# fergusfinn/qmps

Hardware: AMD Instinct MI355X
Metric: two-site energy evals/sec at D=4, batch=65536 (higher is better)
Workload: dtype f64

## Files before the change

### qmps_amd/csrc/qmps_direct.hip

```cpp
#include <hip/hip_runtime.h>
#include <stdint.h>

#include "qmps_hip.h"
#include "qmps_kernels.h"
#include "qmps_device.h"
#include "qmps_circuit.h"
#include "qmps_direct_core.h"
#include "qmps_direct_d8.h"

namespace qmps {

namespace {

struct QuadOps {
  using V = double;
  using P = bool;
  int q;
  const double2* row;
  double* gj;
  __device__ __forceinline__ P q_eq(int i) const { return q == i; }
  __device__ __forceinline__ P q_gt(int i) const { return q > i; }
  template <int L>
  static __device__ __forceinline__ V bcast(V v) { return quad_bcast<L>(v); }
  template <int L, int K>
  __device__ __forceinline__ void row_bcast(const V (&r)[16], V (&out)[16]) const {
#ifdef QMPS_GJ_LDS
    constexpr int K0 = K & ~1;
    __builtin_amdgcn_wave_barrier();
    if (q == L) {
#pragma unroll
      for (int j = K0; j < 16; j += 2) *(double2*)&gj[j] = make_double2(r[j], r[j + 1]);
    }
    __builtin_amdgcn_wave_barrier();
#pragma unroll
    for (int j = K0; j < 16; j += 2) {
      const double2 t = *(const double2*)&gj[j];
      if (j >= K) out[j] = t.x;
      out[j + 1] = t.y;
    }
#else
#pragma unroll
    for (int j = K; j < 16; ++j) out[j] = quad_bcast<L>(r[j]);
#endif
  }
  static __device__ __forceinline__ V qsum(V v) { return quad_sum(v); }
  static __device__ __forceinline__ V qmax(V v) {
    v = fmax(v, quad_perm<0xB1>(v));
    return fmax(v, quad_perm<0x4E>(v));
  }
  static __device__ __forceinline__ V vabs(V v) { return fabs(v); }
  static __device__ __forceinline__ V vmax(V a, V b) { return fmax(a, b); }
  static __device__ __forceinline__ V sel(P p, V a, V b) { return p ? a : b; }
  static __device__ __forceinline__ V splat(double x) { return x; }
  static __device__ __forceinline__ V fma(V a, V b, V c) { return dfma(a, b, c); }
  static __device__ __forceinline__ V rcp(V t) { return fast_rcp(t); }
  static __device__ __forceinline__ P lt(V a, V b) { return a < b; }
  static __device__ __forceinline__ P gt0(V a) { return a > 0.0; }
  static __device__ __forceinline__ P p_and(P a, P b) { return a && b; }
  static __device__ __forceinline__ P p_not(P a) { return !a; }
  static __device__ __forceinline__ bool any(P a) { return __any(a) != 0; }
  __device__ __forceinline__ void own(int s, int j, V& re, V& im) const {
    const double2 v = row[(4 * s + q) * 4 + j];
    re = v.x;
    im = v.y;
  }
  __device__ __forceinline__ void uni(int s, int i, int j, V& re, V& im) const {
    const double2 v = row[(4 * s + i) * 4 + j];
    re = v.x;
    im = v.y;
  }
  __device__ __forceinline__ void col(int s, int i, V& re, V& im) const {
    const double2 v = row[(4 * s + i) * 4 + q];
    re = v.x;
    im = v.y;
  }
};

typedef const __attribute__((address_space(4))) double* const_f64_ptr;
__device__ __forceinline__ const_f64_ptr h_term(const void* h, int t) { return (const_f64_ptr)(uintptr_t)h + 32 * t; }

typedef double v4f64 __attribute__((ext_vector_type(4)));
constexpr int kSqLD = 17;
constexpr int kSqDoubles = 16 * kSqLD + 16;

__device__ __forceinline__ void squaring_fallback(const unsigned char* tiles, int pad, double* img, int lane, bool todo,
                                                  int max_iter, double tol2, double (&x)[4], double& steps, bool& left) {
  constexpr int D = 4, LD = kSqLD;
  constexpr double RS2 = 0.70710678118654752, S2 = 1.4142135623730951;
  const int g = lane >> 4, c = lane & 15, j = c >> 2, jp = c & 3, q = lane & 3;
  double* strip = img + 16 * LD;
  const double cpx = j == jp ? 1.0 : (j < jp ? RS2 : 0.0), cpy = j > jp ? -RS2 : 0.0;
  const double cqx = j < jp ? RS2 : 0.0, cqy = j > jp ? RS2 : 0.0;
  const bool diag = j == jp;
  unsigned long long mask = __ballot(todo);
  while (mask != 0) {
    const int e = (__ffsll((long long)mask) - 1) >> 2;
    mask &= ~(0xFull << (4 * e));
    const double2* sA = (const double2*)(tiles + e * pad);
    v4f64 R;
    {
      double pr[2], pi[2], qr[2], qi[2];
#pragma unroll
      for (int s = 0; s < 2; ++s) {
        const double2 a = sA[(s * D + g) * D + jp], b = sA[(s * D + g) * D + j];
        pr[s] = dfma(cpx, a.x, cpy * a.y);
        pi[s] = dfma(cpy, a.x, -cpx * a.y);
        qr[s] = dfma(cqx, b.x, cqy * b.y);
        qi[s] = dfma(cqy, b.x, -cqx * b.y);
      }
#pragma unroll
      for (int reg = 0; reg < 4; ++reg) {
        double gr = 0.0, gi = 0.0;
#pragma unroll
        for (int s = 0; s < 2; ++s) {
          const double2 u = sA[(s * D + reg) * D + j], v = sA[(s * D + reg) * D + jp];
          gr = dfma(u.x, pr[s], gr);
          gr = dfma(-u.y, pi[s], gr);
          gr = dfma(v.x, qr[s], gr);
          gr = dfma(-v.y, qi[s], gr);
          gi = dfma(u.x, pi[s], gi);
          gi = dfma(u.y, pr[s], gi);
          gi = dfma(v.x, qi[s], gi);
          gi = dfma(v.y, qr[s], gi);
        }
        R[reg] = reg == g ? gr : (reg < g ? S2 * gr : -S2 * gi);
      }
    }
    double af[4];
    auto image = [&](const v4f64& M) {
      __builtin_amdgcn_wave_barrier();
#pragma unroll
      for (int reg = 0; reg < 4; ++reg) img[(4 * reg + g) * LD + c] = M[reg];
      __builtin_amdgcn_wave_barrier();
#pragma unroll
      for (int kk = 0; kk < 4; ++kk) af[kk] = img[c * LD + 4 * kk + g];
    };
    image(R);
    double prev = diag ? 0.25 : 0.0, z = prev, st = 0.0;
    bool active = true;
    int m = 0;
    while (active && m < 29 && (2 << m) <= max_iter) {
      v4f64 acc = {0.0, 0.0, 0.0, 0.0};
#pragma unroll
      for (int kk = 0; kk < 4; ++kk) acc = __builtin_amdgcn_mfma_f64_16x16x4f64(af[kk], R[kk], acc, 0, 0, 0);
      ++m;
      image(acc);
      z = 0.25 * ((img[c * LD + 0] + img[c * LD + 5]) + (img[c * LD + 10] + img[c * LD + 15]));
      const double inv = fast_rcp(row16_sum(diag ? z : 0.0));
      z *= inv;
      R = acc * inv;
#pragma unroll
      for (int kk = 0; kk < 4; ++kk) af[kk] *= inv;
      const double d = z - prev;
      const double d2 = row16_sum(d * d);
      prev = z;
      st = (double)(1 << m);
      active = !(d2 < tol2);
    }
    __builtin_amdgcn_wave_barrier();
    if (lane < 16) strip[lane] = diag ? z : RS2 * z;
    __builtin_amdgcn_wave_barrier();
    if ((lane >> 2) == e) {
      if (m > 0) {
#pragma unroll
        for (int l = 0; l < 4; ++l) x[l] = strip[4 * q + l];
      }
      steps = 1.0 + st;
      left = active;
    }
  }
}

}

#ifndef QMPS_DIRECT_MINWAVES
#define QMPS_DIRECT_MINWAVES 2
#endif
template <int ANS, bool WARM>
__global__ __launch_bounds__(64, QMPS_DIRECT_MINWAVES) void energy_direct_d4_kernel(LaneArgs p) {
  using Core = DirectD4<QuadOps>;
  constexpr int ROW = 512, PAD = ROW + 16, ITEMS = 16;
  __shared__ __attribute__((aligned(16))) unsigned char lds[ITEMS * PAD];
  __shared__ double sq_img[kSqDoubles];
#ifdef QMPS_GJ_LDS
  __shared__ __attribute__((aligned(16))) double gjbuf[ITEMS * 18];
#endif
  const int lane = threadIdx.x, e = lane >> 2, q = lane & 3;
  const int64_t first = (int64_t)blockIdx.x * ITEMS;
  const int64_t b = first + e;
  const bool valid = b < p.B;
  if constexpr (ANS >= 0) {
    Reg<3> reg;
#pragma unroll
    for (int xx = 0; xx < 8; ++xx) {
      reg.re[xx] = (valid && xx == q) ? 1.0 : 0.0;
      reg.im[xx] = 0.0;
    }
    const int nsh = p.ans_nsh;
    const int64_t row = valid ? b : 0;
    const int64_t ridx = nsh > 0 ? row / nsh : row;
    const int shift_k = nsh > 0 ? (int)(row - ridx * nsh) : 0;
    const int isel = nsh > 0 ? *p.ans_i : -1;
    const double* pp = p.ans_params + ridx * p.ans_P;
    constexpr int per = ANS == QMPS_ANSATZ_SHALLOW_CNOT3 ? 3 : 2, trip = ANS == QMPS_ANSATZ_SHALLOW_CNOT3 ? 3 : 4;
    const int P = p.ans_P;
    for (int l = 0; l + per <= P; l += trip) {
      const int mine = l + q;
      double ang = 0.0;
      if (q < trip && mine < P) {
        ang = pp[mine];
        if (mine == isel) ang += roto_shift_value(nsh, shift_k);
      }
      const double scale = ansatz_angle_scale<ANS>(ANS == QMPS_ANSATZ_SHALLOW_CNOT3 ? q : (q & 1));
      double sn, cs;
      sincos(scale * ang, &sn, &cs);
      {
        const double c0[3] = {quad_bcast<0>(cs), quad_bcast<1>(cs), quad_bcast<2>(cs)};
        const double s0[3] = {quad_bcast<0>(sn), quad_bcast<1>(sn), quad_bcast<2>(sn)};
        ansatz_layer_cs<3, ANS>(reg, c0, s0);
      }
      if (trip == 4 && l + 2 + per <= P) {
        const double c1[2] = {quad_bcast<2>(cs), quad_bcast<3>(cs)};
        const double s1[2] = {quad_bcast<2>(sn), quad_bcast<3>(sn)};
        ansatz_layer_cs<3, ANS>(reg, c1, s1);
      }
    }
    double2* tile = (double2*)(lds + e * PAD);
#pragma unroll
    for (int xx = 0; xx < 8; ++xx) tile[((xx & 1) * 4 + (xx >> 1)) * 4 + q] = make_double2(reg.re[xx], reg.im[xx]);
  } else {
    const unsigned char* slab = (const unsigned char*)p.A + first * ROW;
    const int64_t slab_bytes = (p.B - first < ITEMS ? p.B - first : ITEMS) * (int64_t)ROW;
    double2 v[ITEMS * ROW / 1024];
#pragma unroll
    for (int c = 0; c < ITEMS * ROW / 1024; ++c) {
      const int off = c * 1024 + lane * 16;
      v[c] = make_double2(0.0, 0.0);
      if (off < slab_bytes) v[c] = *(const double2*)(slab + off);
    }
#pragma unroll
    for (int c = 0; c < ITEMS * ROW / 1024; ++c) {
      const int off = c * 1024 + lane * 16;
      *(double2*)(lds + (off / ROW) * PAD + (off % ROW)) = v[c];
    }
  }
  __syncthreads();
#ifdef QMPS_GJ_LDS
  const QuadOps o{q, (const double2*)(lds + e * PAD), gjbuf + e * 18};
#else
  const QuadOps o{q, (const double2*)(lds + e * PAD), nullptr};
#endif
  const double tol2 = p.tol * p.tol;

  double x[4], us[16];
  double steps = 1.0;
  int status = QMPS_ST_OK;
  [[maybe_unused]] Core::SiteW W;
  bool have = false;
  if constexpr (WARM) {
    const double2* rin = (const double2*)p.r_in + (valid ? b : 0) * 16;
#pragma unroll
    for (int l = 0; l < 4; ++l) {
      const double2 rw = rin[q * 4 + l], cl = rin[l * 4 + q];
      x[l] = q <= l ? rw.x : cl.y;
    }
    Core::normalise(o, x);
    Core::gather(x, us);
    double y[4];
    const double d2 = Core::power_step(o, x, us, y);
    have = valid && d2 < tol2;
#pragma unroll
    for (int l = 0; l < 4; ++l) x[l] = have ? y[l] : x[l];
    __builtin_amdgcn_sched_barrier(0);
  }
  if (!WARM || __any(valid && !have)) {
    double Rc[4][16], xs[4], y[4];
    Core::build(o, Rc);
    __builtin_amdgcn_sched_barrier(0);
    double pivmax;
    Core::solve(o, Rc, xs, pivmax);
    __builtin_amdgcn_sched_barrier(0);
    Core::normalise(o, xs);
    Core::gather(xs, us);
    double d2;
    if constexpr (WARM) d2 = Core::power_step(o, xs, us, y);
    else d2 = Core::power_step_sites(o, xs, us, p.rho_need, y, W);
    __builtin_amdgcn_sched_barrier(0);
    const bool accepted = d2 < tol2 && pivmax < Core::kMaxInversePivot;
    if (!have) {
#pragma unroll
      for (int l = 0; l < 4; ++l) x[l] = xs[l];
      if (WARM) steps = 2.0;
    }
    const bool todo = valid && !have && !accepted;
    if (__any(todo)) {
      bool left = false;
      squaring_fallback(lds, PAD, sq_img, lane, todo, p.max_iter - 1, tol2, x, steps, left);
      if (__any(todo && left)) {
        double yb[4];
        Core::gather(x, us);
        const double d2b = Core::power_step(o, x, us, yb);
        const bool fin = todo && left && d2b < tol2 && steps + 1.0 <= (double)p.max_iter;
#pragma unroll
        for (int l = 0; l < 4; ++l) x[l] = fin ? yb[l] : x[l];
        if (fin) {
          left = false;
          steps += 1.0;
        }
      }
      if (todo) {
        status = left ? QMPS_ST_NOT_CONVERGED : QMPS_ST_OK;
        if (WARM) steps += 1.0;
      }
      if constexpr (!WARM) {
        Core::gather(x, us);
        Core::update_sites(o, us, p.rho_need, todo, W);
      }
    }
    if constexpr (WARM) Core::gather(x, us);
  } else {
    Core::gather(x, us);
  }
  __builtin_amdgcn_sched_barrier(0);

  double pre[4][4], pim[4][4];
  bool pd;
  if constexpr (WARM) pd = Core::density(o, us, p.rho_need, pre, pim);
  else pd = Core::density_sites(o, us, p.rho_need, W, pre, pim);
  if (status == QMPS_ST_OK && !pd) status = QMPS_ST_NOT_PD;
  if (p.acc_zero != nullptr && blockIdx.x == 0) acc_clear(p.acc_zero, p.n_terms, lane, 64);
  for (int t = 0; t < p.n_terms; ++t) {
    const double en = quad_sum(Core::energy(h_term(p.h, t), p.rho_need, pre, pim));
    if (valid && q == 0) p.E[b * p.n_terms + t] = en;
    if (p.partial != nullptr || p.acc != nullptr) {
      const double s = wave_sum((valid && q == 0) ? en : 0.0);
      if (lane == 0) {
        if (p.partial != nullptr) p.partial[(int64_t)t * gridDim.x + blockIdx.x] = s;
        if (p.acc != nullptr) acc_arrive(p.acc, p.acc_shards, t, blockIdx.x, s, p.acc_bound, p.acc_scale);
      }
    }
  }
  if (p.rho_out != nullptr) {
    double fre[4][4], fim[4][4];
#pragma unroll
    for (int t = 0; t < 4; ++t)
#pragma unroll
      for (int s = t; s < 4; ++s) {
        fre[t][s] = quad_sum(pre[t][s]);
        fim[t][s] = t == s ? 0.0 : quad_sum(pim[t][s]);
      }
    if (valid && q == 0) {
      double2* o2 = (double2*)p.rho_out + b * 16;
#pragma unroll
      for (int t = 0; t < 4; ++t)
#pragma unroll
        for (int s = 0; s < 4; ++s)
          o2[t * 4 + s] = t <= s ? make_double2(fre[t][s], fim[t][s]) : make_double2(fre[s][t], -fim[s][t]);
    }
  }
  if (!valid) return;
  if (q == 0) {
    p.iters[b] = (int32_t)steps;
    p.status[b] = status;
  }
  if (p.r_out != nullptr) {
    double2* o2 = (double2*)p.r_out + b * 16 + q * 4;
#pragma unroll
    for (int l = 0; l < 4; ++l) {
      const double f = q == 0 ? us[4 * l] : (q == 1 ? us[4 * l + 1] : (q == 2 ? us[4 * l + 2] : us[4 * l + 3]));
      const double re = q <= l ? x[l] : f;
      const double im = q == l ? 0.0 : (q < l ? f : -x[l]);
      o2[l] = make_double2(re, im);
    }
  }
}

#ifndef QMPS_ENERGY_ONLY_LEAN_WAVES
#define QMPS_ENERGY_ONLY_LEAN_WAVES 2
#endif
template <bool LEAN>
__global__ __launch_bounds__(64, LEAN ? QMPS_ENERGY_ONLY_LEAN_WAVES : 2) void energy_only_d4_kernel(LaneArgs p) {
  using Core = DirectD4<QuadOps>;
  constexpr int ROW = 512, PAD = ROW + 16, ITEMS = 16;
  __shared__ __attribute__((aligned(16))) unsigned char lds[ITEMS * PAD];
  const int lane = threadIdx.x, e = lane >> 2, q = lane & 3;
  const int64_t first = (int64_t)blockIdx.x * ITEMS;
  const int64_t b = first + e;
  const bool valid = b < p.B;
  if (p.acc_zero != nullptr && blockIdx.x == 0) acc_clear(p.acc_zero, p.n_terms, lane, 64);
  {
    const unsigned char* slab = (const unsigned char*)p.A + first * ROW;
    const int64_t slab_bytes = (p.B - first < ITEMS ? p.B - first : ITEMS) * (int64_t)ROW;
    double2 v[ITEMS * ROW / 1024];
#pragma unroll
    for (int c = 0; c < ITEMS * ROW / 1024; ++c) {
      const int off = c * 1024 + lane * 16;
      v[c] = make_double2(0.0, 0.0);
      if (off < slab_bytes) v[c] = *(const double2*)(slab + off);
    }
    double x[4];
    {
      const double2* rin = (const double2*)p.r_in + (valid ? b : 0) * 16;
#pragma unroll
      for (int l = 0; l < 4; ++l) {
        const double2 rw = rin[q * 4 + l], cl = rin[l * 4 + q];
        x[l] = q <= l ? rw.x : cl.y;
      }
    }
#pragma unroll
    for (int c = 0; c < ITEMS * ROW / 1024; ++c) {
      const int off = c * 1024 + lane * 16;
      *(double2*)(lds + (off / ROW) * PAD + (off % ROW)) = v[c];
    }
    __syncthreads();
    const QuadOps o{q, (const double2*)(lds + e * PAD), nullptr};
    Core::normalise(o, x);
    double us[16];
    double pre[4][4], pim[4][4], bre[4][4], bim[4][4];
    bool pd = true;
    if constexpr (LEAN) {
      Core::b_rows(o, bre, bim);
      Core::gather(x, us);
    } else {
      Core::gather(x, us);
      pd = Core::density(o, us, p.rho_need, pre, pim);
    }
    int status = QMPS_ST_OK;
    if (p.check_pd) {
      status = valid ? p.status[b] : QMPS_ST_OK;
      if (status == QMPS_ST_OK && !pd) status = QMPS_ST_NOT_PD;
    }
    for (int t = 0; t < p.n_terms; ++t) {
      double en;
      if constexpr (LEAN) en = quad_sum(Core::energy_lean(bre, bim, us, (const double*)p.h + 32 * t));
      else en = quad_sum(Core::energy(h_term(p.h, t), p.rho_need, pre, pim));
      if (valid && q == 0) p.E[b * p.n_terms + t] = en;
      if (p.partial != nullptr || p.acc != nullptr) {
        const double s = wave_sum((valid && q == 0) ? en : 0.0);
        if (lane == 0) {
          if (p.partial != nullptr) p.partial[(int64_t)t * gridDim.x + blockIdx.x] = s;
          if (p.acc != nullptr) acc_arrive(p.acc, p.acc_shards, t, blockIdx.x, s, p.acc_bound, p.acc_scale);
        }
      }
    }
    if (!LEAN && p.rho_out != nullptr) {
      double fre[4][4], fim[4][4];
#pragma unroll
      for (int t = 0; t < 4; ++t)
#pragma unroll
        for (int s2 = t; s2 < 4; ++s2) {
          fre[t][s2] = quad_sum(pre[t][s2]);
          fim[t][s2] = t == s2 ? 0.0 : quad_sum(pim[t][s2]);
        }
      if (valid && q == 0) {
        double2* o2 = (double2*)p.rho_out + b * 16;
#pragma unroll
        for (int t = 0; t < 4; ++t)
#pragma unroll
          for (int s2 = 0; s2 < 4; ++s2)
            o2[t * 4 + s2] = t <= s2 ? make_double2(fre[t][s2], fim[t][s2]) : make_double2(fre[s2][t], -fim[s2][t]);
      }
    }
    if (p.check_pd && valid && q == 0) p.status[b] = status;
  }
}

#ifndef QMPS_POWER_D4_MINWAVES
#define QMPS_POWER_D4_MINWAVES 4
#endif
template <int B, bool FRESH = false>
__device__ __forceinline__ void row_fmac(double& acc, double u, double m) {
  if constexpr (FRESH) asm("s_nop 1\n\tv_fmac_f64_dpp %0, %1, %2 row_newbcast:%3 row_mask:0xf bank_mask:0xf" : "+v"(acc) : "v"(u), "v"(m), "n"(B));
  else asm("v_fmac_f64_dpp %0, %1, %2 row_newbcast:%3 row_mask:0xf bank_mask:0xf" : "+v"(acc) : "v"(u), "v"(m), "n"(B));
}
template <bool GUESS>
__global__ __launch_bounds__(64, QMPS_POWER_D4_MINWAVES) void env_power_d4_kernel(LaneArgs p, int* __restrict__ counter, int first_block) {
  constexpr int PAD = 512 + 16, SLOTS = 4, kChunk = 8;
  __shared__ __attribute__((aligned(16))) unsigned char lds[SLOTS * PAD];
  const int lane = threadIdx.x, g = lane >> 4, c = lane & 15, i = c >> 2, ip = c & 3;
  const bool diag = i == ip, rot = i > ip;
  const double wt = diag ? 1.0 : 2.0;
  const double tol2 = p.tol * p.tol;
  const unsigned long long below = (1ull << (lane & ~15)) - 1ull;
  const double2* tile = (const double2*)(lds + g * PAD);
  int64_t b = 0;
  const int64_t dyn0 = (int64_t)gridDim.x * first_block;
  int64_t next = (int64_t)blockIdx.x * first_block, end = next + first_block;
  if (next > p.B) next = p.B;
  if (end > p.B) end = p.B;
  bool active = false, exhausted = dyn0 >= p.B;
  bool refill = true;
  int iters = 0;
  double u = 0.0, up = 0.0, R[16];
#pragma unroll
  for (int k = 0; k < 16; ++k) R[k] = 0.0;
  for (;;) {
    if (refill) {
      const unsigned long long idle = __ballot(!active);
      if (idle != 0ull && !(exhausted && next >= end)) {
        if (next >= end && !exhausted) {
          int base = 0;
          if (lane == 0) base = atomicAdd(counter, kChunk);
          const int64_t first = dyn0 + (int64_t)__builtin_amdgcn_readfirstlane(base);
          next = first < p.B ? first : p.B;
          end = first + kChunk < p.B ? first + kChunk : p.B;
          exhausted = first + kChunk >= p.B;
        }
        const int64_t nb = next + (__popcll(idle & below) >> 4);
        const int64_t lim = end;
        {
          const int64_t take = (int64_t)(__popcll(idle) >> 4);
          next = next + take < end ? next + take : end;
        }
        if (!active && nb < lim) {
          b = nb;
          {
            const double2* src = (const double2*)p.A + b * 32;
            const double2 v0 = src[c], v1 = src[c + 16];
            double2* w = (double2*)(lds + g * PAD);
            w[c] = v0;
            w[c + 16] = v1;
          }
          __builtin_amdgcn_wave_barrier();
          double tr[2][4], ti[2][4], br[2][4], bi[2][4];
#pragma unroll
          for (int s = 0; s < 2; ++s)
#pragma unroll
            for (int j = 0; j < 4; ++j) {
              const double2 a = tile[(4 * s + i) * 4 + j], cc = tile[(4 * s + ip) * 4 + j];
              tr[s][j] = rot ? -a.y : a.x;
              ti[s][j] = rot ? a.x : a.y;
              br[s][j] = cc.x;
              bi[s][j] = cc.y;
            }
#pragma unroll
          for (int j = 0; j < 4; ++j) {
            double v = tr[0][j] * br[0][j];
            v = dfma(ti[0][j], bi[0][j], v);
            v = dfma(tr[1][j], br[1][j], v);
            v = dfma(ti[1][j], bi[1][j], v);
            R[5 * j] = v;
          }
#pragma unroll
          for (int lo = 0; lo < 4; ++lo)
#pragma unroll
            for (int hi = lo + 1; hi < 4; ++hi) {
              double re = tr[0][lo] * br[0][hi], im = tr[0][lo] * bi[0][hi];
#pragma unroll
              for (int s = 0; s < 2; ++s) {
                if (s > 0) {
                  re = dfma(tr[s][lo], br[s][hi], re);
                  im = dfma(tr[s][lo], bi[s][hi], im);
                }
                re = dfma(ti[s][lo], bi[s][hi], re);
                re = dfma(tr[s][hi], br[s][lo], re);
                re = dfma(ti[s][hi], bi[s][lo], re);
                im = dfma(-ti[s][lo], br[s][hi], im);
                im = dfma(ti[s][hi], br[s][lo], im);
                im = dfma(-tr[s][hi], bi[s][lo], im);
              }
              R[4 * lo + hi] = re;
              R[4 * hi + lo] = im;
            }
          u = diag ? 0.25 : 0.0;
          if constexpr (GUESS) {
            const double2* rin = (const double2*)p.r_in + b * 16;
            const double2 rw = rin[4 * i + ip], cl = rin[4 * ip + i];
            const double ug = i <= ip ? 0.5 * (rw.x + cl.x) : 0.5 * (cl.y - rw.y);
            const double t = row16_sum(diag ? ug : 0.0);
            const bool usable = t > 1e-300 && t < 1e300;
            if (usable) u = ug * (1.0 / t);
          }
          up = u;
          iters = 0;
          active = true;
        }
      }
      const unsigned long long still = __ballot(!active);
      if (still == ~0ull) break;
      refill = still != 0ull && !(exhausted && next >= end);
    }
    double y0 = 0.0, y1 = 0.0, y2 = 0.0, y3 = 0.0;
    row_fmac<0, true>(y0, u, R[0]); row_fmac<1>(y1, u, R[1]);   row_fmac<2>(y2, u, R[2]);   row_fmac<3>(y3, u, R[3]);
    row_fmac<4>(y0, u, R[4]);       row_fmac<5>(y1, u, R[5]);   row_fmac<6>(y2, u, R[6]);   row_fmac<7>(y3, u, R[7]);
    row_fmac<8>(y0, u, R[8]);       row_fmac<9>(y1, u, R[9]);   row_fmac<10>(y2, u, R[10]); row_fmac<11>(y3, u, R[11]);
    row_fmac<12>(y0, u, R[12]);     row_fmac<13>(y1, u, R[13]); row_fmac<14>(y2, u, R[14]); row_fmac<15>(y3, u, R[15]);
    const double d = u - up;
    const double d2 = row16_sum(wt * d * d);
    const double y = (y0 + y1) + (y2 + y3);
    double t0 = 0.0, t1 = 0.0;
    row_fmac<0, true>(t0, y, 1.0); row_fmac<5>(t1, y, 1.0); row_fmac<10>(t0, y, 1.0); row_fmac<15>(t1, y, 1.0);
    const double yn = y * fast_rcp(t0 + t1);
    const bool conv = iters > 0 && d2 < tol2;
    const bool fin = active && (conv || iters >= p.max_iter);
    if (__any(fin)) {
      if (fin) {
        if (c == 0) {
          p.iters[b] = iters;
          p.status[b] = conv ? QMPS_ST_OK : QMPS_ST_NOT_CONVERGED;
        }
        const double ut = __shfl(u, (lane & ~15) + 4 * ip + i, 64);
        const double re = i <= ip ? u : ut;
        const double im = diag ? 0.0 : (i < ip ? ut : -u);
        ((double2*)p.r_out)[b * 16 + c] = make_double2(re, im);
        active = false;
      }
      refill = true;
    }
    iters = active ? iters + 1 : iters;
    up = active ? u : up;
    u = active ? yn : u;
  }
}

hipError_t launch_env_power_d4(const LaneArgs& a, int* counter, int waves, hipStream_t st) {
  if (a.B <= 0) return hipSuccess;
  if (a.r_out == nullptr || counter == nullptr) return hipErrorInvalidValue;
  const int64_t need = (a.B + 3) / 4;
  const int64_t nw = need < waves ? need : (waves < 1 ? 1 : waves);
  const dim3 grid((unsigned)nw), block(64);
  int first_block = (int)(a.B / (2 * nw) / 4 * 4);
  if (first_block < 4) first_block = 4;
  if (a.r_in != nullptr) hipLaunchKernelGGL(env_power_d4_kernel<true>, grid, block, 0, st, a, counter, first_block);
  else hipLaunchKernelGGL(env_power_d4_kernel<false>, grid, block, 0, st, a, counter, first_block);
  return hipGetLastError();
}

hipError_t launch_energy_only_d4(const LaneArgs& a, hipStream_t st) {
  if (a.B <= 0) return hipSuccess;
  const dim3 grid((unsigned)((a.B + 15) / 16)), block(64);
  if (a.rho_out == nullptr && !a.check_pd && a.n_terms <= 2) hipLaunchKernelGGL(energy_only_d4_kernel<true>, grid, block, 0, st, a);
  else hipLaunchKernelGGL(energy_only_d4_kernel<false>, grid, block, 0, st, a);
  return hipGetLastError();
}

__global__ __launch_bounds__(64) void cost_finish_kernel(const long long* __restrict__ acc, int n_shards, long long expect,
                                                         int max_polls, double inv_scale, int n_terms,
                                                         double* __restrict__ cost, int* __restrict__ err) {
  const int lane = threadIdx.x;
  for (int t = 0; t < n_terms; ++t) {
    double cnt = 0.0, hi = 0.0, lo = 0.0;
    for (int poll = 0;; ++poll) {
      long long c_i = 0, hi_i = 0, lo_i = 0;
      for (int i = lane; i < n_shards; i += 64) {
        const long long w = __hip_atomic_load(acc + t * kAccMaxShards + i, __ATOMIC_RELAXED, __HIP_MEMORY_SCOPE_AGENT);
        long long c, v;
        acc_decode(w, c, v);
        c_i += c;
        hi_i += v >> 20;
        lo_i += v & 0xFFFFF;
      }
      cnt = wave_sum((double)c_i);
      hi = wave_sum((double)hi_i);
      lo = wave_sum((double)lo_i);
      if (expect <= 0 || cnt >= (double)expect || poll >= max_polls) break;
      __builtin_amdgcn_s_sleep(32);
    }
    if (lane == 0) {
      const bool ok = expect <= 0 || cnt == (double)expect;
      const double over = __hip_atomic_load((const double*)(acc + kAccOver) + t, __ATOMIC_RELAXED, __HIP_MEMORY_SCOPE_AGENT);
      cost[t] = ok ? (hi * 1048576.0 + lo) * inv_scale + over : __builtin_nan("");
      if (!ok && err != nullptr) *err = 1;
    }
  }
}

hipError_t launch_cost_finish(const long long* acc, int n_shards, long long expect, int max_polls, double inv_scale,
                              int n_terms, double* cost, int* err, hipStream_t st) {
  hipLaunchKernelGGL(cost_finish_kernel, dim3(1), dim3(64), 0, st, acc, n_shards, expect, max_polls, inv_scale, n_terms, cost, err);
  return hipGetLastError();
}

__global__ __launch_bounds__(64, 2) void env_direct_d8_kernel(const double2* __restrict__ A, double2* __restrict__ r_out, int64_t B) {
  constexpr int D = 8, N = 64, P = D + 1;
  __shared__ double2 sA[2][D][P];
  __shared__ double sT[D][P];
  __shared__ double sM[N][17];
  const int lane = threadIdx.x, i = lane >> 3, ip = lane & 7;
  const int64_t b = blockIdx.x;
  if (b >= B) return;
  {
    const double2* a = A + b * (2 * N);
    sA[0][i][ip] = a[lane];
    sA[1][i][ip] = a[N + lane];
  }
  __builtin_amdgcn_wave_barrier();
  __syncthreads();
  r_out[b * N + lane] = env_direct_d8_solve(sA, sT, sM, lane);
}

hipError_t launch_env_direct_d8(const void* A, void* r_out, int64_t B, hipStream_t st) {
  if (B <= 0) return hipSuccess;
  hipLaunchKernelGGL(env_direct_d8_kernel, dim3((unsigned)B), dim3(64), 0, st, (const double2*)A, (double2*)r_out, B);
  return hipGetLastError();
}

hipError_t launch_energy_direct_d4(const LaneArgs& a, hipStream_t st) {
  if (a.B <= 0) return hipSuccess;
  const dim3 grid((unsigned)((a.B + 15) / 16)), block(64);
  const bool warm = a.r_in != nullptr;
  if (a.ans_params == nullptr) {
    if (warm) hipLaunchKernelGGL((energy_direct_d4_kernel<-1, true>), grid, block, 0, st, a);
    else hipLaunchKernelGGL((energy_direct_d4_kernel<-1, false>), grid, block, 0, st, a);
  } else if (warm) {
    switch (a.ans_kind) {
      case QMPS_ANSATZ_SHALLOW_CNOT: hipLaunchKernelGGL((energy_direct_d4_kernel<QMPS_ANSATZ_SHALLOW_CNOT, true>), grid, block, 0, st, a); break;
      case QMPS_ANSATZ_SHALLOW_QAOA: hipLaunchKernelGGL((energy_direct_d4_kernel<QMPS_ANSATZ_SHALLOW_QAOA, true>), grid, block, 0, st, a); break;
      case QMPS_ANSATZ_SHALLOW_CNOT3: hipLaunchKernelGGL((energy_direct_d4_kernel<QMPS_ANSATZ_SHALLOW_CNOT3, true>), grid, block, 0, st, a); break;
      default: return hipErrorInvalidValue;
    }
  } else {
    switch (a.ans_kind) {
      case QMPS_ANSATZ_SHALLOW_CNOT: hipLaunchKernelGGL((energy_direct_d4_kernel<QMPS_ANSATZ_SHALLOW_CNOT, false>), grid, block, 0, st, a); break;
      case QMPS_ANSATZ_SHALLOW_QAOA: hipLaunchKernelGGL((energy_direct_d4_kernel<QMPS_ANSATZ_SHALLOW_QAOA, false>), grid, block, 0, st, a); break;
      case QMPS_ANSATZ_SHALLOW_CNOT3: hipLaunchKernelGGL((energy_direct_d4_kernel<QMPS_ANSATZ_SHALLOW_CNOT3, false>), grid, block, 0, st, a); break;
      default: return hipErrorInvalidValue;
    }
  }
  return hipGetLastError();
}

}
```

### qmps_amd/csrc/qmps_direct_core.h

```cpp
#pragma once

#include <stdint.h>

#include <utility>

namespace qmps {

constexpr uint32_t kRhoNeedAll = 0xFFFFFFFFu;
inline uint32_t rho_need_mask(const double* h, int n_terms) {
  uint32_t need = 0;
  for (int n = 0; n < n_terms; ++n)
    for (int s = 0; s < 4; ++s)
      for (int t = 0; t < 4; ++t) {
        const int lo = t < s ? t : s, hi = t < s ? s : t;
        const double re = h[32 * n + 2 * (4 * s + t)], im = h[32 * n + 2 * (4 * s + t) + 1];
        if (!(re == 0.0)) need |= 1u << (4 * lo + hi);
        if (lo != hi && !(im == 0.0)) need |= 1u << (16 + 4 * lo + hi);
      }
  return need;
}

constexpr uint32_t kSiteN00 = 1u, kSiteN10 = 2u, kSiteN11 = 4u, kSiteW01 = 8u, kSiteW10 = 16u;
constexpr uint32_t rho_site_parts(uint32_t factor) {
  uint32_t parts = 0;
  for (int tau = 0; tau < 4; ++tau)
    for (int sg = tau; sg < 4; ++sg) {
      const int t1 = tau >> 1, t2 = tau & 1, s1 = sg >> 1, s2 = sg & 1;
      const uint32_t n = s1 == 0 ? kSiteN00 : (t1 == 0 ? kSiteN10 : kSiteN11);
      const uint32_t w = t2 == s2 ? 0u : (t2 == 0 ? kSiteW01 : kSiteW10);
      if (factor == n || factor == w) parts |= (1u << (4 * tau + sg)) | (sg != tau ? 1u << (16 + 4 * tau + sg) : 0u);
    }
  return parts;
}
constexpr uint32_t rho_site_factors(uint32_t need) {
  return ((need & rho_site_parts(kSiteN00)) != 0u ? kSiteN00 : 0u) | ((need & rho_site_parts(kSiteN10)) != 0u ? kSiteN10 : 0u) |
         ((need & rho_site_parts(kSiteN11)) != 0u ? kSiteN11 : 0u) | ((need & rho_site_parts(kSiteW01)) != 0u ? kSiteW01 : 0u) |
         ((need & rho_site_parts(kSiteW10)) != 0u ? kSiteW10 : 0u);
}

#if defined(__HIPCC__)
#define QMPS_CORE_FN __device__ inline __attribute__((always_inline))
#define QMPS_SCHED_FENCE() __builtin_amdgcn_sched_barrier(0)
#else
#define QMPS_CORE_FN inline __attribute__((always_inline))
#define QMPS_SCHED_FENCE() ((void)0)
#endif
#if defined(__HIP_DEVICE_COMPILE__)
#define QMPS_COMPUTED_HERE(v) asm volatile("" : "+v"(v))
#else
#define QMPS_COMPUTED_HERE(v) ((void)0)
#endif

template <int... I, class F>
QMPS_CORE_FN void static_for_impl(std::integer_sequence<int, I...>, F&& f) {
  (f(std::integral_constant<int, I>{}), ...);
}
template <int N, class F>
QMPS_CORE_FN void static_for(F&& f) {
  static_for_impl(std::make_integer_sequence<int, N>{}, static_cast<F&&>(f));
}

template <class O>
struct DirectD4 {
  using V = typename O::V;
  using P = typename O::P;

  static QMPS_CORE_FN V own_diag(const O& o, const V (&x)[4]) {
    return O::sel(o.q_eq(0), x[0], O::sel(o.q_eq(1), x[1], O::sel(o.q_eq(2), x[2], x[3])));
  }

  static QMPS_CORE_FN void build(const O& o, V (&Rc)[4][16]) {
    V ar[2][4], ai[2][4];
#pragma unroll
    for (int s = 0; s < 2; ++s)
#pragma unroll
      for (int j = 0; j < 4; ++j) o.own(s, j, ar[s][j], ai[s][j]);
#pragma unroll
    for (int ip = 0; ip < 4; ++ip) {
      const P rot = o.q_gt(ip);
      V tr[2][4], ti[2][4], br[2][4], bi[2][4];
#pragma unroll
      for (int s = 0; s < 2; ++s)
#pragma unroll
        for (int j = 0; j < 4; ++j) {
          tr[s][j] = ip == 3 ? ar[s][j] : O::sel(rot, -ai[s][j], ar[s][j]);
          ti[s][j] = ip == 3 ? ai[s][j] : O::sel(rot, ar[s][j], ai[s][j]);
          o.uni(s, ip, j, br[s][j], bi[s][j]);
        }
#pragma unroll
      for (int j = 0; j < 4; ++j) {
        V v = tr[0][j] * br[0][j];
        v = O::fma(ti[0][j], bi[0][j], v);
        v = O::fma(tr[1][j], br[1][j], v);
        v = O::fma(ti[1][j], bi[1][j], v);
        Rc[ip][5 * j] = v;
      }
#pragma unroll
      for (int lo = 0; lo < 4; ++lo)
#pragma unroll
        for (int hi = lo + 1; hi < 4; ++hi) {
          V re = tr[0][lo] * br[0][hi], im = tr[0][lo] * bi[0][hi];
#pragma unroll
          for (int s = 0; s < 2; ++s) {
            if (s > 0) {
              re = O::fma(tr[s][lo], br[s][hi], re);
              im = O::fma(tr[s][lo], bi[s][hi], im);
            }
            re = O::fma(ti[s][lo], bi[s][hi], re);
            re = O::fma(tr[s][hi], br[s][lo], re);
            re = O::fma(ti[s][hi], bi[s][lo], re);
            im = O::fma(-ti[s][lo], br[s][hi], im);
            im = O::fma(ti[s][hi], br[s][lo], im);
            im = O::fma(-tr[s][hi], bi[s][lo], im);
          }
          Rc[ip][4 * lo + hi] = re;
          Rc[ip][4 * hi + lo] = im;
        }
    }
  }

  static QMPS_CORE_FN void solve(const O& o, V (&M)[4][16], V (&x)[4], V& pivmax) {
    V y[4], dinv[4];
    const V one = O::splat(1.0), zero = O::splat(0.0);
    V w[4];
#pragma unroll
    for (int l = 0; l < 4; ++l) w[l] = O::sel(o.q_eq(l), one, zero);
#pragma unroll
    for (int r = 0; r < 4; ++r) {
#pragma unroll
      for (int l = 0; l < 4; ++l) M[r][4 * l + r] = M[r][4 * l + r] - w[l];
      dinv[r] = zero;
    }
#pragma unroll
    for (int j = 0; j < 4; ++j) M[3][5 * j] = M[3][5 * j] + w[3];
    static_for<16>([&](auto K) {
      constexpr int k = decltype(K)::value, pl = k >> 2, pr = k & 3;
      V prow[16];
      o.template row_bcast<pl, k>(M[pr], prow);
      const V pinv = O::rcp(prow[k]);
      const P mine = o.q_eq(pl);
      dinv[pr] = O::sel(mine, pinv, dinv[pr]);
#pragma unroll
      for (int r = 0; r < 4; ++r) {
        V f = M[r][k] * pinv;
        if (r == pr) f = O::sel(mine, zero, f);
#pragma unroll
        for (int j = k + 1; j < 16; ++j) M[r][j] = O::fma(-f, prow[j], M[r][j]);
        if (k == 15) y[r] = -f;
      }
    });
    y[3] = O::sel(o.q_eq(3), one, y[3]);
#pragma unroll
    for (int r = 0; r < 4; ++r) x[r] = y[r] * dinv[r];
    pivmax = O::qmax(O::vmax(O::vmax(O::vabs(dinv[0]), O::vabs(dinv[1])), O::vmax(O::vabs(dinv[2]), O::vabs(dinv[3]))));
  }

  static constexpr double kMaxInversePivot = 1e10;

  static QMPS_CORE_FN void gather(const V (&x)[4], V (&xs)[16]) {
    static_for<4>([&](auto L) {
      constexpr int l = decltype(L)::value;
#pragma unroll
      for (int r = 0; r < 4; ++r) xs[4 * l + r] = O::template bcast<l>(x[r]);
    });
  }

  static QMPS_CORE_FN V normalise(const O& o, V (&x)[4]) {
    const V tr = O::qsum(own_diag(o, x));
    const V inv = O::rcp(tr);
#pragma unroll
    for (int r = 0; r < 4; ++r) x[r] = x[r] * inv;
    return inv;
  }

  static QMPS_CORE_FN V dist2(const O& o, const V (&x)[4], const V (&y)[4]) {
    V d = O::splat(0.0);
#pragma unroll
    for (int r = 0; r < 4; ++r) {
      const V dd = y[r] - x[r];
      const V wt = O::sel(o.q_eq(r), O::splat(1.0), O::splat(2.0));
      d = O::fma(wt * dd, dd, d);
    }
    return O::qsum(d);
  }

  static QMPS_CORE_FN V power_step(const O& o, const V (&x)[4], const V (&us)[16], V (&y)[4]) {
    V xr[2][4], xi[2][4];
    own_rows_times_r(o, us, xr, xi);
#pragma unroll
    for (int l = 0; l < 4; ++l) {
      V cr = O::splat(0.0), ci = O::splat(0.0);
#pragma unroll
      for (int s = 0; s < 2; ++s)
#pragma unroll
        for (int k = 0; k < 4; ++k) {
          V br, bi;
          o.uni(s, l, k, br, bi);
          cr = O::fma(xr[s][k], br, cr);
          cr = O::fma(xi[s][k], bi, cr);
          ci = O::fma(xi[s][k], br, ci);
          ci = O::fma(-xr[s][k], bi, ci);
        }
      y[l] = l == 3 ? cr : O::sel(o.q_gt(l), -ci, cr);
    }
    normalise(o, y);
    return dist2(o, x, y);
  }
  static QMPS_CORE_FN void own_rows_times_r(const O& o, const V (&us)[16], V (&xr)[2][4], V (&xi)[2][4]) {
    V ar[2][4], ai[2][4];
#pragma unroll
    for (int s = 0; s < 2; ++s)
#pragma unroll
      for (int j = 0; j < 4; ++j) o.own(s, j, ar[s][j], ai[s][j]);
#pragma unroll
    for (int s = 0; s < 2; ++s)
#pragma unroll
      for (int l = 0; l < 4; ++l) {
        V cr = O::splat(0.0), ci = O::splat(0.0);
#pragma unroll
        for (int k = 0; k < 4; ++k) {
          const V rr = us[k <= l ? 4 * k + l : 4 * l + k];
          cr = O::fma(ar[s][k], rr, cr);
          ci = O::fma(ai[s][k], rr, ci);
          if (k != l) {
            const V ri = k < l ? us[4 * l + k] : -us[4 * k + l];
            cr = O::fma(-ai[s][k], ri, cr);
            ci = O::fma(ar[s][k], ri, ci);
          }
        }
        xr[s][l] = cr;
        xi[s][l] = ci;
      }
  }

  struct SiteW {
    V re[2][2][4], im[2][2][4];
  };
  static QMPS_CORE_FN V power_step_sites(const O& o, const V (&x)[4], const V (&us)[16], uint32_t need, V (&y)[4], SiteW& w) {
    V xr[2][4], xi[2][4];
    own_rows_times_r(o, us, xr, xi);
    site_w(o, xr[0], xi[0], 0, w.re[0][0], w.im[0][0]);
    site_w(o, xr[1], xi[1], 1, w.re[1][1], w.im[1][1]);
#pragma unroll
    for (int l = 0; l < 4; ++l) {
      const V cr = w.re[0][0][l] + w.re[1][1][l];
      y[l] = l == 3 ? cr : O::sel(o.q_gt(l), -(w.im[0][0][l] + w.im[1][1][l]), cr);
    }
    const uint32_t f = rho_site_factors(need);
    if (f & kSiteW01) site_w(o, xr[0], xi[0], 1, w.re[0][1], w.im[0][1]);
    if (f & kSiteW10) site_w(o, xr[1], xi[1], 0, w.re[1][0], w.im[1][0]);
    normalise(o, y);
    return dist2(o, x, y);
  }
  static QMPS_CORE_FN void site_w(const O& o, const V (&xr)[4], const V (&xi)[4], int s2, V (&wre)[4], V (&wim)[4]) {
#pragma unroll
    for (int l = 0; l < 4; ++l) {
      V br, bi;
      o.uni(s2, l, 0, br, bi);
      V cr = O::fma(xi[0], bi, xr[0] * br), ci = O::fma(-xr[0], bi, xi[0] * br);
#pragma unroll
      for (int k = 1; k < 4; ++k) {
        o.uni(s2, l, k, br, bi);
        cr = O::fma(xr[k], br, cr);
        cr = O::fma(xi[k], bi, cr);
        ci = O::fma(xi[k], br, ci);
        ci = O::fma(-xr[k], bi, ci);
      }
      wre[l] = cr;
      wim[l] = ci;
    }
  }
  static QMPS_CORE_FN void update_sites(const O& o, const V (&us)[16], uint32_t need, P p, SiteW& w) {
    V xr[2][4], xi[2][4];
    own_rows_times_r(o, us, xr, xi);
    const uint32_t f = rho_site_factors(need);
#pragma unroll
    for (int t2 = 0; t2 < 2; ++t2)
#pragma unroll
      for (int s2 = 0; s2 < 2; ++s2) {
        if (t2 != s2 && !(f & (t2 == 0 ? kSiteW01 : kSiteW10))) continue;
        V tre[4], tim[4];
        site_w(o, xr[t2], xi[t2], s2, tre, tim);
#pragma unroll
        for (int l = 0; l < 4; ++l) {
          w.re[t2][s2][l] = O::sel(p, tre[l], w.re[t2][s2][l]);
          w.im[t2][s2][l] = O::sel(p, tim[l], w.im[t2][s2][l]);
        }
      }
  }

  static QMPS_CORE_FN void square(V (&Rc)[4][16]) {
    V out[4][16];
    static_for<16>([&](auto C) {
      constexpr int c = decltype(C)::value, cl = c >> 2, cr = c & 3;
      V rowc[16];
#pragma unroll
      for (int j = 0; j < 16; ++j) rowc[j] = O::template bcast<cl>(Rc[cr][j]);
#pragma unroll
      for (int r = 0; r < 4; ++r)
#pragma unroll
        for (int j = 0; j < 16; ++j) out[r][j] = c == 0 ? Rc[r][c] * rowc[j] : O::fma(Rc[r][c], rowc[j], out[r][j]);
      QMPS_SCHED_FENCE();
    });
#pragma unroll
    for (int r = 0; r < 4; ++r)
#pragma unroll
      for (int j = 0; j < 16; ++j) Rc[r][j] = out[r][j];
  }

  static QMPS_CORE_FN P squaring(const O& o, V (&Rc)[4][16], P active, int max_iter, double tol2, V (&x)[4], V& steps) {
    V prev[4];
#pragma unroll
    for (int r = 0; r < 4; ++r) prev[r] = O::sel(o.q_eq(r), O::splat(0.25), O::splat(0.0));
    int m = 0;
    while (O::any(active) && m < 29 && (2 << m) <= max_iter) {
      square(Rc);
      ++m;
      V z[4];
#pragma unroll
      for (int r = 0; r < 4; ++r) z[r] = O::splat(0.25) * ((Rc[r][0] + Rc[r][5]) + (Rc[r][10] + Rc[r][15]));
      const V inv = normalise(o, z);
#pragma unroll
      for (int r = 0; r < 4; ++r)
#pragma unroll
        for (int j = 0; j < 16; ++j) Rc[r][j] = Rc[r][j] * inv;
      const P conv = O::lt(dist2(o, prev, z), O::splat(tol2));
#pragma unroll
      for (int r = 0; r < 4; ++r) {
        x[r] = O::sel(active, z[r], x[r]);
        prev[r] = z[r];
      }
      steps = O::sel(active, O::splat((double)(1 << m)), steps);
      active = O::p_and(active, O::p_not(conv));
    }
    return active;
  }

  static QMPS_CORE_FN void b_rows(const O& o, V (&bre)[4][4], V (&bim)[4][4]) {
    V ar[2][4], ai[2][4];
#pragma unroll
    for (int s = 0; s < 2; ++s)
#pragma unroll
      for (int j = 0; j < 4; ++j) o.own(s, j, ar[s][j], ai[s][j]);
#pragma unroll
    for (int t2 = 0; t2 < 2; ++t2)
#pragma unroll
      for (int j = 0; j < 4; ++j) {
        V ur[4], ui[4];
#pragma unroll
        for (int k = 0; k < 4; ++k) o.uni(t2, j, k, ur[k], ui[k]);
#pragma unroll
        for (int t1 = 0; t1 < 2; ++t1)
#pragma unroll
          for (int k = 0; k < 4; ++k) {
            V cr, ci;
            if (j == 0) {
              cr = ar[t1][0] * ur[k];
              ci = ar[t1][0] * ui[k];
            } else {
              cr = O::fma(ar[t1][j], ur[k], bre[2 * t1 + t2][k]);
              ci = O::fma(ar[t1][j], ui[k], bim[2 * t1 + t2][k]);
            }
            bre[2 * t1 + t2][k] = O::fma(-ai[t1][j], ui[k], cr);
            bim[2 * t1 + t2][k] = O::fma(ai[t1][j], ur[k], ci);
          }
      }
  }

  static QMPS_CORE_FN V energy_lean(const V (&bre)[4][4], const V (&bim)[4][4], const V (&us)[16], const double* h) {
    V e = O::splat(0.0);
#pragma unroll
    for (int sg = 0; sg < 4; ++sg) {
      V cr[4], ci[4];
#pragma unroll
      for (int l = 0; l < 4; ++l) {
        cr[l] = O::splat(0.0);
        ci[l] = O::splat(0.0);
      }
#pragma unroll
      for (int tau = 0; tau < 4; ++tau) {
        const V hr = O::splat(h[2 * (4 * sg + tau)]), hi = O::splat(h[2 * (4 * sg + tau) + 1]);
#pragma unroll
        for (int l = 0; l < 4; ++l) {
          cr[l] = O::fma(hr, bre[tau][l], cr[l]);
          cr[l] = O::fma(-hi, bim[tau][l], cr[l]);
          ci[l] = O::fma(hr, bim[tau][l], ci[l]);
          ci[l] = O::fma(hi, bre[tau][l], ci[l]);
        }
      }
#pragma unroll
      for (int l = 0; l < 4; ++l) {
        V zr = O::splat(0.0), zi = O::splat(0.0);
#pragma unroll
        for (int k = 0; k < 4; ++k) {
          const V rr = us[k <= l ? 4 * k + l : 4 * l + k];
          zr = O::fma(cr[k], rr, zr);
          zi = O::fma(ci[k], rr, zi);
          if (k != l) {
            const V ri = k < l ? us[4 * l + k] : -us[4 * k + l];
            zr = O::fma(-ci[k], ri, zr);
            zi = O::fma(cr[k], ri, zi);
          }
        }
        e = O::fma(zr, bre[sg][l], e);
        e = O::fma(zi, bim[sg][l], e);
      }
    }
    return e;
  }

  static QMPS_CORE_FN P ldl(const V (&us)[16], V (&rre)[4][4], V (&rim)[4][4], V (&lre)[4][4], V (&lim)[4][4], V (&d)[4]) {
#pragma unroll
    for (int k = 0; k < 4; ++k)
#pragma unroll
      for (int l = k; l < 4; ++l) {
        rre[k][l] = us[4 * k + l];
        rim[k][l] = k == l ? O::splat(0.0) : us[4 * l + k];
      }
    P pd = O::gt0(rre[0][0]);
#pragma unroll
    for (int j = 0; j < 4; ++j) {
      V dj = rre[j][j];
#pragma unroll
      for (int k = 0; k < j; ++k) dj = O::fma(-(lre[j][k] * lre[j][k] + lim[j][k] * lim[j][k]), d[k], dj);
      d[j] = dj;
      pd = O::p_and(pd, O::gt0(dj));
      const V inv = O::rcp(O::sel(O::gt0(dj), dj, O::splat(1.0)));
#pragma unroll
      for (int i = j + 1; i < 4; ++i) {
        V cr = rre[j][i], ci = -rim[j][i];
#pragma unroll
        for (int k = 0; k < j; ++k) {
          const V pr = lre[i][k] * lre[j][k] + lim[i][k] * lim[j][k];
          const V pi = lim[i][k] * lre[j][k] - lre[i][k] * lim[j][k];
          cr = O::fma(-pr, d[k], cr);
          ci = O::fma(-pi, d[k], ci);
        }
        lre[i][j] = cr * inv;
        lim[i][j] = ci * inv;
      }
    }
    return pd;
  }

  static QMPS_CORE_FN P density(const O& o, const V (&us)[16], V (&pre)[4][4], V (&pim)[4][4]) {
    return density(o, us, kRhoNeedAll, pre, pim);
  }
  static QMPS_CORE_FN P density(const O& o, const V (&us)[16], uint32_t need, V (&pre)[4][4], V (&pim)[4][4]) {
    V rre[4][4], rim[4][4], lre[4][4], lim[4][4], d[4];
    const P pd = ldl(us, rre, rim, lre, lim, d);
    V bre[4][4], bim[4][4];
    b_rows(o, bre, bim);
#pragma unroll
    for (int tau = 0; tau < 4; ++tau)
#pragma unroll
      for (int k = 0; k < 4; ++k) {
        V cr = bre[tau][k], ci = bim[tau][k];
#pragma unroll
        for (int i = k + 1; i < 4; ++i) {
          cr = O::fma(bre[tau][i], lre[i][k], cr);
          cr = O::fma(-bim[tau][i], lim[i][k], cr);
          ci = O::fma(bre[tau][i], lim[i][k], ci);
          ci = O::fma(bim[tau][i], lre[i][k], ci);
        }
        bre[tau][k] = cr;
        bim[tau][k] = ci;
      }
    computed_here(bre, bim);
#pragma unroll
    for (int tau = 0; tau < 4; ++tau) {
      V gre[4], gim[4];
#pragma unroll
      for (int k = 0; k < 4; ++k) {
        gre[k] = bre[tau][k] * d[k];
        gim[k] = bim[tau][k] * d[k];
      }
      rho_row(tau, need, gre, gim, bre, bim, pre, pim);
    }
    QMPS_SCHED_FENCE();
    if (O::any(O::p_not(pd))) {
      b_rows(o, bre, bim);
      computed_here(bre, bim);
#pragma unroll
      for (int tau = 0; tau < 4; ++tau) {
        V yre[4], yim[4];
#pragma unroll
        for (int l = 0; l < 4; ++l) {
          V cr = O::splat(0.0), ci = O::splat(0.0);
#pragma unroll
          for (int k = 0; k < 4; ++k) {
            const V rr = k <= l ? rre[k][l] : rre[l][k];
            cr = O::fma(bre[tau][k], rr, cr);
            ci = O::fma(bim[tau][k], rr, ci);
            if (k != l) {
              const V ri = k < l ? rim[k][l] : -rim[l][k];
              cr = O::fma(-bim[tau][k], ri, cr);
              ci = O::fma(bre[tau][k], ri, ci);
            }
          }
          yre[l] = cr;
          yim[l] = ci;
          QMPS_COMPUTED_HERE(yre[l]);
          QMPS_COMPUTED_HERE(yim[l]);
        }
        V qre[4][4], qim[4][4];
        rho_row(tau, need, yre, yim, bre, bim, qre, qim);
#pragma unroll
        for (int sg = tau; sg < 4; ++sg) {
          pre[tau][sg] = O::sel(pd, pre[tau][sg], qre[tau][sg]);
          pim[tau][sg] = O::sel(pd, pim[tau][sg], qim[tau][sg]);
        }
      }
      QMPS_SCHED_FENCE();
    }
    return pd;
  }

  static QMPS_CORE_FN void computed_here(V (&bre)[4][4], V (&bim)[4][4]) {
#pragma unroll
    for (int tau = 0; tau < 4; ++tau)
#pragma unroll
      for (int k = 0; k < 4; ++k) {
        QMPS_COMPUTED_HERE(bre[tau][k]);
        QMPS_COMPUTED_HERE(bim[tau][k]);
      }
  }

  static QMPS_CORE_FN void rho_row(int tau, const V (&yre)[4], const V (&yim)[4], const V (&bre)[4][4], const V (&bim)[4][4],
                                   V (&pre)[4][4], V (&pim)[4][4]) {
    rho_row(tau, kRhoNeedAll, yre, yim, bre, bim, pre, pim);
  }
  static QMPS_CORE_FN void rho_row(int tau, uint32_t need, const V (&yre)[4], const V (&yim)[4], const V (&bre)[4][4],
                                   const V (&bim)[4][4], V (&pre)[4][4], V (&pim)[4][4]) {
#pragma unroll
    for (int sg = tau; sg < 4; ++sg) {
      V cr = O::splat(0.0);
      if ((need >> (4 * tau + sg)) & 1u) {
        cr = yre[0] * bre[sg][0];
        cr = O::fma(yim[0], bim[sg][0], cr);
#pragma unroll
        for (int l = 1; l < 4; ++l) {
          cr = O::fma(yre[l], bre[sg][l], cr);
          cr = O::fma(yim[l], bim[sg][l], cr);
        }
      }
      pre[tau][sg] = cr;
      pim[tau][sg] = O::splat(0.0);
    }
    if ((need >> (16 + 4 * tau)) & 0xFu) {
#pragma unroll
      for (int sg = tau + 1; sg < 4; ++sg)
        if ((need >> (16 + 4 * tau + sg)) & 1u) {
          V ci = O::splat(0.0);
#pragma unroll
          for (int l = 0; l < 4; ++l) {
            ci = O::fma(yim[l], bre[sg][l], ci);
            ci = O::fma(-yre[l], bim[sg][l], ci);
          }
          pim[tau][sg] = ci;
        }
    }
  }

  static QMPS_CORE_FN P density_sites(const O& o, const V (&us)[16], uint32_t need, const SiteW& w, V (&pre)[4][4], V (&pim)[4][4]) {
    P pd;
    {
      V rre[4][4], rim[4][4], lre[4][4], lim[4][4], d[4];
      pd = ldl(us, rre, rim, lre, lim, d);
    }
#pragma unroll
    for (int tau = 0; tau < 4; ++tau)
#pragma unroll
      for (int sg = tau; sg < 4; ++sg) {
        pre[tau][sg] = O::splat(0.0);
        pim[tau][sg] = O::splat(0.0);
      }
    static_for<3>([&](auto F) {
      constexpr int s1 = decltype(F)::value == 0 ? 0 : 1, t1 = decltype(F)::value == 2 ? 1 : 0;
      constexpr uint32_t parts = rho_site_parts(1u << decltype(F)::value);
      if (need & parts) {
        V cr[4], ci[4], nre[4], nim[4];
#pragma unroll
        for (int i = 0; i < 4; ++i) o.col(t1, i, cr[i], ci[i]);
#pragma unroll
        for (int l = 0; l < 4; ++l) {
          V ur, ui;
          o.uni(s1, 0, l, ur, ui);
          V re = O::fma(ui, ci[0], ur * cr[0]), im = O::fma(-ui, cr[0], ur * ci[0]);
#pragma unroll
          for (int i = 1; i < 4; ++i) {
            o.uni(s1, i, l, ur, ui);
            re = O::fma(ur, cr[i], re);
            re = O::fma(ui, ci[i], re);
            im = O::fma(ur, ci[i], im);
            im = O::fma(-ui, cr[i], im);
          }
          nre[l] = re;
          nim[l] = im;
        }
#pragma unroll
        for (int l = 0; l < 4; ++l) {
          QMPS_COMPUTED_HERE(nre[l]);
          QMPS_COMPUTED_HERE(nim[l]);
        }
#pragma unroll
        for (int t2 = 0; t2 < 2; ++t2)
#pragma unroll
          for (int s2 = 0; s2 < 2; ++s2) {
            const int tau = 2 * t1 + t2, sg = 2 * s1 + s2;
            if (tau > sg) continue;
            if ((need >> (4 * tau + sg)) & 1u) {
              V c = w.re[t2][s2][0] * nre[0];
              c = O::fma(-w.im[t2][s2][0], nim[0], c);
#pragma unroll
              for (int l = 1; l < 4; ++l) {
                c = O::fma(w.re[t2][s2][l], nre[l], c);
                c = O::fma(-w.im[t2][s2][l], nim[l], c);
              }
              pre[tau][sg] = c;
            }
          }
        if ((need & parts) >> 16) {
#pragma unroll
          for (int t2 = 0; t2 < 2; ++t2)
#pragma unroll
            for (int s2 = 0; s2 < 2; ++s2) {
              const int tau = 2 * t1 + t2, sg = 2 * s1 + s2;
              if (tau >= sg) continue;
              if ((need >> (16 + 4 * tau + sg)) & 1u) {
                V c = w.re[t2][s2][0] * nim[0];
                c = O::fma(w.im[t2][s2][0], nre[0], c);
#pragma unroll
                for (int l = 1; l < 4; ++l) {
                  c = O::fma(w.re[t2][s2][l], nim[l], c);
                  c = O::fma(w.im[t2][s2][l], nre[l], c);
                }
                pim[tau][sg] = c;
              }
            }
        }
      }
    });
    QMPS_SCHED_FENCE();
    return pd;
  }

  static QMPS_CORE_FN V energy(const double* h, const V (&pre)[4][4], const V (&pim)[4][4]) {
    return energy(h, kRhoNeedAll, pre, pim);
  }
  template <class H>
  static QMPS_CORE_FN V energy(H h, uint32_t need, const V (&pre)[4][4], const V (&pim)[4][4]) {
    V e = O::splat(0.0);
    if ((need >> 16) != 0u) {
#pragma unroll
      for (int s = 0; s < 4; ++s) {
#pragma unroll
        for (int t = 0; t < 4; ++t) {
          const double hr = h[2 * (4 * s + t)], hi = h[2 * (4 * s + t) + 1];
          const V rr = t <= s ? pre[t][s] : pre[s][t];
          e = O::fma(O::splat(hr), rr, e);
          if (t != s) {
            const V ri = t < s ? pim[t][s] : -pim[s][t];
            e = O::fma(O::splat(-hi), ri, e);
          }
        }
        QMPS_COMPUTED_HERE(e);
      }
    } else {
#pragma unroll
      for (int s = 0; s < 4; ++s)
#pragma unroll
        for (int t = 0; t < 4; ++t) e = O::fma(O::splat(h[2 * (4 * s + t)]), t <= s ? pre[t][s] : pre[s][t], e);
    }
    return e;
  }
};

}
```

Measured before the change: 2.372 billion.

## Replace Gauss-Jordan solve with Gaussian elimination plus broadcast back-substitution

Rewrites the 16x16 linear solve spread across a lane quad. It switches from full Gauss-Jordan elimination, which updates every row at each pivot, to forward elimination below the pivot followed by back-substitution that broadcasts each solved coordinate. The solution comes out already gathered across the quad, so the separate normalise and gather steps are fused into a cheap trace-based normalisation. The aim is fewer FMAs and quad broadcasts per solve, at the cost of a serial back-substitution chain. The unused LDS row-broadcast variant is removed.

```diff
diff --git a/qmps_amd/csrc/qmps_direct.hip b/qmps_amd/csrc/qmps_direct.hip
--- a/qmps_amd/csrc/qmps_direct.hip
+++ b/qmps_amd/csrc/qmps_direct.hip
@@ -17,32 +17,10 @@
   using P = bool;
   int q;
   const double2* row;
-  double* gj;
   __device__ __forceinline__ P q_eq(int i) const { return q == i; }
   __device__ __forceinline__ P q_gt(int i) const { return q > i; }
   template <int L>
   static __device__ __forceinline__ V bcast(V v) { return quad_bcast<L>(v); }
-  template <int L, int K>
-  __device__ __forceinline__ void row_bcast(const V (&r)[16], V (&out)[16]) const {
-#ifdef QMPS_GJ_LDS
-    constexpr int K0 = K & ~1;
-    __builtin_amdgcn_wave_barrier();
-    if (q == L) {
-#pragma unroll
-      for (int j = K0; j < 16; j += 2) *(double2*)&gj[j] = make_double2(r[j], r[j + 1]);
-    }
-    __builtin_amdgcn_wave_barrier();
-#pragma unroll
-    for (int j = K0; j < 16; j += 2) {
-      const double2 t = *(const double2*)&gj[j];
-      if (j >= K) out[j] = t.x;
-      out[j + 1] = t.y;
-    }
-#else
-#pragma unroll
-    for (int j = K; j < 16; ++j) out[j] = quad_bcast<L>(r[j]);
-#endif
-  }
   static __device__ __forceinline__ V qsum(V v) { return quad_sum(v); }
   static __device__ __forceinline__ V qmax(V v) {
     v = fmax(v, quad_perm<0xB1>(v));
@@ -182,9 +160,6 @@
   constexpr int ROW = 512, PAD = ROW + 16, ITEMS = 16;
   __shared__ __attribute__((aligned(16))) unsigned char lds[ITEMS * PAD];
   __shared__ double sq_img[kSqDoubles];
-#ifdef QMPS_GJ_LDS
-  __shared__ __attribute__((aligned(16))) double gjbuf[ITEMS * 18];
-#endif
   const int lane = threadIdx.x, e = lane >> 2, q = lane & 3;
   const int64_t first = (int64_t)blockIdx.x * ITEMS;
   const int64_t b = first + e;
@@ -245,11 +220,7 @@
     }
   }
   __syncthreads();
-#ifdef QMPS_GJ_LDS
-  const QuadOps o{q, (const double2*)(lds + e * PAD), gjbuf + e * 18};
-#else
-  const QuadOps o{q, (const double2*)(lds + e * PAD), nullptr};
-#endif
+  const QuadOps o{q, (const double2*)(lds + e * PAD)};
   const double tol2 = p.tol * p.tol;
 
   double x[4], us[16];
@@ -278,10 +249,12 @@
     Core::build(o, Rc);
     __builtin_amdgcn_sched_barrier(0);
     double pivmax;
-    Core::solve(o, Rc, xs, pivmax);
-    __builtin_amdgcn_sched_barrier(0);
-    Core::normalise(o, xs);
-    Core::gather(xs, us);
+    {
+      double ur[16];
+      Core::solve_gathered(o, Rc, ur, pivmax);
+      __builtin_amdgcn_sched_barrier(0);
+      Core::normalise_gathered(o, ur, us, xs);
+    }
     double d2;
     if constexpr (WARM) d2 = Core::power_step(o, xs, us, y);
     else d2 = Core::power_step_sites(o, xs, us, p.rho_need, y, W);
@@ -413,7 +386,7 @@
       *(double2*)(lds + (off / ROW) * PAD + (off % ROW)) = v[c];
     }
     __syncthreads();
-    const QuadOps o{q, (const double2*)(lds + e * PAD), nullptr};
+    const QuadOps o{q, (const double2*)(lds + e * PAD)};
     Core::normalise(o, x);
     double us[16];
     double pre[4][4], pim[4][4], bre[4][4], bim[4][4];
diff --git a/qmps_amd/csrc/qmps_direct_core.h b/qmps_amd/csrc/qmps_direct_core.h
--- a/qmps_amd/csrc/qmps_direct_core.h
+++ b/qmps_amd/csrc/qmps_direct_core.h
@@ -119,8 +119,10 @@
     }
   }
 
-  static QMPS_CORE_FN void solve(const O& o, V (&M)[4][16], V (&x)[4], V& pivmax) {
-    V y[4], dinv[4];
+  static constexpr int piv_coord(int k) { return 4 * (k & 3) + (k >> 2); }
+
+  static QMPS_CORE_FN void solve_gathered(const O& o, V (&M)[4][16], V (&ur)[16], V& pivmax) {
+    V dinv[4];
     const V one = O::splat(1.0), zero = O::splat(0.0);
     V w[4];
 #pragma unroll
@@ -134,25 +136,56 @@
 #pragma unroll
     for (int j = 0; j < 4; ++j) M[3][5 * j] = M[3][5 * j] + w[3];
     static_for<16>([&](auto K) {
-      constexpr int k = decltype(K)::value, pl = k >> 2, pr = k & 3;
+      constexpr int k = decltype(K)::value, pl = k & 3, pr = k >> 2, a = piv_coord(k);
       V prow[16];
-      o.template row_bcast<pl, k>(M[pr], prow);
-      const V pinv = O::rcp(prow[k]);
-      const P mine = o.q_eq(pl);
-      dinv[pr] = O::sel(mine, pinv, dinv[pr]);
-#pragma unroll
-      for (int r = 0; r < 4; ++r) {
-        V f = M[r][k] * pinv;
-        if (r == pr) f = O::sel(mine, zero, f);
-#pragma unroll
-        for (int j = k + 1; j < 16; ++j) M[r][j] = O::fma(-f, prow[j], M[r][j]);
-        if (k == 15) y[r] = -f;
+      prow[a] = O::template bcast<pl>(M[pr][a]);
+#pragma unroll
+      for (int k2 = k + 1; k2 < 16; ++k2) prow[piv_coord(k2)] = O::template bcast<pl>(M[pr][piv_coord(k2)]);
+      const V pinv = O::rcp(prow[a]);
+      dinv[pr] = O::sel(o.q_eq(pl), pinv, dinv[pr]);
+      if (pl < 3) {
+        const V f = O::sel(o.q_gt(pl), M[pr][a] * pinv, zero);
+#pragma unroll
+        for (int k2 = k + 1; k2 < 16; ++k2) M[pr][piv_coord(k2)] = O::fma(-f, prow[piv_coord(k2)], M[pr][piv_coord(k2)]);
+      }
+#pragma unroll
+      for (int r = pr + 1; r < 4; ++r) {
+        const V f = M[r][a] * pinv;
+#pragma unroll
+        for (int k2 = k + 1; k2 < 16; ++k2) M[r][piv_coord(k2)] = O::fma(-f, prow[piv_coord(k2)], M[r][piv_coord(k2)]);
       }
     });
-    y[3] = O::sel(o.q_eq(3), one, y[3]);
-#pragma unroll
-    for (int r = 0; r < 4; ++r) x[r] = y[r] * dinv[r];
+    V s[4];
+    ur[15] = one;
+    static_for<15>([&](auto J) {
+      constexpr int j = 15 - decltype(J)::value, pl = j & 3, pr = j >> 2, a = piv_coord(j);
+      constexpr int nl = (j - 1) & 3, nr = (j - 1) >> 2;
+#pragma unroll
+      for (int r = pl > 0 ? pr : pr - 1; r >= 0; --r) {
+        if constexpr (j == 15) s[r] = M[r][a];
+        else s[r] = O::fma(M[r][a], ur[a], s[r]);
+      }
+      ur[piv_coord(j - 1)] = O::template bcast<nl>((-s[nr]) * dinv[nr]);
+    });
     pivmax = O::qmax(O::vmax(O::vmax(O::vabs(dinv[0]), O::vabs(dinv[1])), O::vmax(O::vabs(dinv[2]), O::vabs(dinv[3]))));
+  }
+
+  static QMPS_CORE_FN void own_coords(const O& o, const V (&us)[16], V (&x)[4]) {
+#pragma unroll
+    for (int r = 0; r < 4; ++r) x[r] = O::sel(o.q_eq(0), us[r], O::sel(o.q_eq(1), us[4 + r], O::sel(o.q_eq(2), us[8 + r], us[12 + r])));
+  }
+
+  static QMPS_CORE_FN void solve(const O& o, V (&M)[4][16], V (&x)[4], V& pivmax) {
+    V ur[16];
+    solve_gathered(o, M, ur, pivmax);
+    own_coords(o, ur, x);
+  }
+
+  static QMPS_CORE_FN void normalise_gathered(const O& o, const V (&ur)[16], V (&us)[16], V (&x)[4]) {
+    const V inv = O::rcp((ur[0] + ur[5]) + (ur[10] + ur[15]));
+#pragma unroll
+    for (int a = 0; a < 16; ++a) us[a] = ur[a] * inv;
+    own_coords(o, us, x);
   }
 
   static constexpr double kMaxInversePivot = 1e10;
```

Result: faster. 2.405 billion, median of 6 (+1.4%).
